# rafaelvp-db/databricks-distributed-deep-learning

Hardware: AMD Instinct MI355X
Metric: ResNet-50 images/sec (whole node) (higher is better)
Workload: dtype bf16

## Files before the change

### csrc/kernels/conv3_bwd.hip

```cpp
#include "ddl_lds.h"

#include <algorithm>

namespace {

constexpr int NW = 8, NTH = NW * 64;
constexpr int TM = 32;
constexpr int DPT = 6, SPT = 1;

struct C3Params {
    const bf16_t* dz;
    const bf16_t* x3;
    const float* mean3;
    const float* istd3;
    const float* coef3;
    const bf16_t* a2;
    const bf16_t* x2;
    const uint8_t* mask2;
    const float* mean2;
    const float* istd2;
    const bf16_t* wt;
    bf16_t* dz2;
    float* colstats;
    bf16_t* wpart;
    long M;
    int tiles, chunk;
    uint32_t dz2_bytes;
};

__device__ __forceinline__ u32x4 bn_apply8(bf16x8 dzv, bf16x8 xv, const float* A, const float* B, const float* D,
                                           bool valid) {
    const u32x4 gw = __builtin_bit_cast(u32x4, dzv), xw = __builtin_bit_cast(u32x4, xv);
    const uint32_t keep = valid ? ~0u : 0u;
    u32x4 o;
#pragma unroll
    for (int i = 0; i < 4; ++i) {
        const float g0 = lo_f(gw[i]), g1 = hi_f(gw[i]);
        const float x0 = lo_f(xw[i]), x1 = hi_f(xw[i]);
        const float o0 = bn_bwd_apply1(A[2 * i], g0, B[2 * i], x0, D[2 * i]);
        const float o1 = bn_bwd_apply1(A[2 * i + 1], g1, B[2 * i + 1], x1, D[2 * i + 1]);
        o[i] = pack2bf(o0, o1) & keep;
    }
    return o;
}

template <int CO, int CI, int NBUF>
__global__ __launch_bounds__(NTH, 1) void conv3_bwd_k(C3Params p) {
    static_assert(CO == 256 && CI == 64 && (NBUF == 2 || NBUF == 3), "shape");
    constexpr int WBYTES = CI * CO * 2, ZBYTES = TM * CO * 2, ABYTES = TM * CI * 2;
    constexpr int O_DZ = 0, O_X3 = ZBYTES, O_A2 = 2 * ZBYTES, O_X2 = O_A2 + ABYTES, O_MK = O_X2 + ABYTES;
    constexpr int BUFB = O_MK + 1024;
    constexpr int LDS = WBYTES + NBUF * BUFB;
    static_assert(LDS <= 160 * 1024, "LDS");
    __shared__ __attribute__((aligned(16))) char smem[LDS];
    const int tid = threadIdx.x, lane = tid & 63, wv = __builtin_amdgcn_readfirstlane(tid >> 6);
    const int g = lane >> 4, r16 = lane & 15;
    const uint32_t lds0 = (uint32_t)(uintptr_t)smem;
    const __amdgpu_buffer_rsrc_t crs = rsrc(p.dz2, p.dz2_bytes);
    const int t0 = blockIdx.x * p.chunk, t1 = min(p.tiles, t0 + p.chunk);

    auto prefetch = [&](int t, int buf) {
        char* base = smem + WBYTES + buf * BUFB;
        const long m0 = (long)t * TM;
#pragma unroll
        for (int qq = 0; qq < 2; ++qq) {
            const int q = qq * NW + wv, r = q * 2 + (lane >> 5), c = (lane & 31) ^ (r & 15);
            const long gr = min(m0 + r, p.M - 1);
            glds16_nt(p.dz + gr * CO + c * 8, base + O_DZ + q * 1024);
            glds16_nt(p.x3 + gr * CO + c * 8, base + O_X3 + q * 1024);
        }
        {
            const int q = wv & 3, r = q * 8 + (lane >> 3), c = (lane & 7) ^ (r & 7);
            const long gr = min(m0 + r, p.M - 1);
            glds16_nt((wv < 4 ? p.a2 : p.x2) + gr * CI + c * 8, base + (wv < 4 ? O_A2 : O_X2) + q * 1024);
        }
        {
            const long b = min(m0 * (CI / 8) + lane * 4, p.M * (CI / 8) - 4);
            const uint8_t* src = p.mask2 ? p.mask2 + b : (const uint8_t*)p.a2;
            glds4(src, base + O_MK);
        }
    };
#pragma unroll
    for (int qq = 0; qq < CI / 2 / NW; ++qq) {
        const int q = qq * NW + wv, r = q * 2 + (lane >> 5), c = (lane & 31) ^ (r & 15);
        glds16_nt(p.wt + (long)r * CO + c * 8, smem + q * 1024);
    }
#pragma unroll
    for (int u = 0; u < NBUF - 1; ++u)
        if (t0 + u < t1) prefetch(t0 + u, u);

    const int tc = tid & 31, tr = tid >> 5;
    float cA[8], cB[8], cD[8];
    bn_bwd_apply_coefs8(p.mean3, p.istd3, p.coef3, CO, tc * 8, cA, cB, cD);
    const uint32_t toff = tr * (CO * 2) + ((tc ^ tr) << 4);

    const int dj = wv & 3;
    const bool dgw = wv < 4;
    uint32_t aoff[2][CO / 32], boff[CO / 32];
#pragma unroll
    for (int kk = 0; kk < CO / 32; ++kk) {
        const int rb = 16 * dj + r16;
        boff[kk] = lds0 + rb * (CO * 2) + (((kk * 4 + g) ^ (rb & 15)) << 4);
#pragma unroll
        for (int i = 0; i < 2; ++i) {
            const int ra = 16 * i + r16;
            aoff[i][kk] = ra * (CO * 2) + (((kk * 4 + g) ^ (ra & 15)) << 4);
        }
    }
    uint32_t coff[2], moff[2];
#pragma unroll
    for (int i = 0; i < 2; ++i) {
        const int drow = 16 * i + r16;
        coff[i] = drow * (CI * 2) + (((2 * dj + (g >> 1)) ^ (drow & 7)) << 4) + (g & 1) * 8;
        moff[i] = drow * (CI / 8) + (dj >> 1) * 4;
    }
    const int mshift = (dj & 1) * 16 + 4 * g;
    float st_s[4] = {0.f, 0.f, 0.f, 0.f}, st_q[4] = {0.f, 0.f, 0.f, 0.f};

    const int q4 = (lane >> 2) & 3, pq = lane & 3;
    uint32_t wa[2][2], wb[4][2];
#pragma unroll
    for (int h = 0; h < 2; ++h) {
        const int r = 8 * g + q4 + 4 * h;
#pragma unroll
        for (int i = 0; i < 2; ++i) {
            const int col = 32 * wv + 16 * i + 4 * pq;
            wa[i][h] = r * (CO * 2) + (((col >> 3) ^ (r & 15)) << 4) + (pq & 1) * 8;
        }
#pragma unroll
        for (int j = 0; j < 4; ++j) {
            const int col = 16 * j + 4 * pq;
            wb[j][h] = r * (CI * 2) + (((col >> 3) ^ (r & 7)) << 4) + (pq & 1) * 8;
        }
    }
    f32x4 wacc[2][4];
#pragma unroll
    for (int i = 0; i < 2; ++i)
#pragma unroll
        for (int j = 0; j < 4; ++j) wacc[i][j] = (f32x4){0.f, 0.f, 0.f, 0.f};

    int buf = 0;
    for (int t = t0; t < t1; ++t) {
        wait_vm(min(NBUF - 1, t - t0) * SPT + min(NBUF - 2, t1 - 1 - t) * DPT);
        __builtin_amdgcn_s_barrier();
        if (t + NBUF - 1 < t1) prefetch(t + NBUF - 1, buf == 0 ? NBUF - 1 : buf - 1);
        const uint32_t img = lds0 + WBYTES + buf * BUFB;
        const long m0 = (long)t * TM;

        {
            const bf16x8 z0 = ds_read16(img + O_DZ + toff), z1 = ds_read16(img + O_DZ + toff + 16 * CO * 2);
            const bf16x8 x0 = ds_read16(img + O_X3 + toff), x1 = ds_read16(img + O_X3 + toff + 16 * CO * 2);
            LGKM0();
            __builtin_amdgcn_sched_barrier(0);
            ds_write16(img + O_DZ + toff, bn_apply8(z0, x0, cA, cB, cD, m0 + tr < p.M));
            ds_write16(img + O_DZ + toff + 16 * CO * 2, bn_apply8(z1, x1, cA, cB, cD, m0 + tr + 16 < p.M));
            LGKM0();
            __builtin_amdgcn_s_barrier();
        }

        f32x4 acc[2] = {{0.f, 0.f, 0.f, 0.f}, {0.f, 0.f, 0.f, 0.f}};
        if (dgw) {
#pragma unroll
            for (int k2 = 0; k2 < CO / 32; k2 += 4) {
                bf16x8 af[2][4], bfr[4];
#pragma unroll
                for (int u = 0; u < 4; ++u) {
                    af[0][u] = ds_read16(img + O_DZ + aoff[0][k2 + u]);
                    af[1][u] = ds_read16(img + O_DZ + aoff[1][k2 + u]);
                    bfr[u] = ds_read16(boff[k2 + u]);
                }
                LGKM0();
                __builtin_amdgcn_sched_barrier(0);
#pragma unroll
                for (int u = 0; u < 4; ++u) {
                    acc[0] = __builtin_amdgcn_mfma_f32_16x16x32_bf16(bfr[u], af[0][u], acc[0], 0, 0, 0);
                    acc[1] = __builtin_amdgcn_mfma_f32_16x16x32_bf16(bfr[u], af[1][u], acc[1], 0, 0, 0);
                }
                __builtin_amdgcn_sched_barrier(0);
            }
        }
        s16x4 fal[2][2], fbl[4][2];
#pragma unroll
        for (int h = 0; h < 2; ++h) {
#pragma unroll
            for (int i = 0; i < 2; ++i) fal[i][h] = ds_read_tr8(img + O_DZ + wa[i][h]);
#pragma unroll
            for (int j = 0; j < 4; ++j) fbl[j][h] = ds_read_tr8(img + O_A2 + wb[j][h]);
        }
        uint32_t mword[2] = {~0u, ~0u};
        uint2 ev[2] = {make_uint2(0u, 0u), make_uint2(0u, 0u)};
        if (dgw) {
#pragma unroll
            for (int i = 0; i < 2; ++i) {
                if (p.mask2) mword[i] = ds_read32(img + O_MK + moff[i]);
                ev[i] = ds_read8(img + O_X2 + coff[i]);
            }
        }
        LGKM0();
        __builtin_amdgcn_sched_barrier(0);
        {
            typedef short s16x8 __attribute__((ext_vector_type(8)));
            bf16x8 fa[2], fb[4];
#pragma unroll
            for (int i = 0; i < 2; ++i) {
                const s16x8 r = {fal[i][0][0], fal[i][0][1], fal[i][0][2], fal[i][0][3],
                                 fal[i][1][0], fal[i][1][1], fal[i][1][2], fal[i][1][3]};
                fa[i] = __builtin_bit_cast(bf16x8, r);
            }
#pragma unroll
            for (int j = 0; j < 4; ++j) {
                const s16x8 r = {fbl[j][0][0], fbl[j][0][1], fbl[j][0][2], fbl[j][0][3],
                                 fbl[j][1][0], fbl[j][1][1], fbl[j][1][2], fbl[j][1][3]};
                fb[j] = __builtin_bit_cast(bf16x8, r);
            }
#pragma unroll
            for (int i = 0; i < 2; ++i)
#pragma unroll
                for (int j = 0; j < 4; ++j)
                    wacc[i][j] = __builtin_amdgcn_mfma_f32_16x16x32_bf16(fb[j], fa[i], wacc[i][j], 0, 0, 0);
        }
        if (dgw) {
#pragma unroll
            for (int i = 0; i < 2; ++i) {
                float v[4] = {acc[i][0], acc[i][1], acc[i][2], acc[i][3]};
                const float xv[4] = {lo_f(ev[i].x), hi_f(ev[i].x), lo_f(ev[i].y), hi_f(ev[i].y)};
                const uint32_t bits = mword[i] >> mshift;
#pragma unroll
                for (int e = 0; e < 4; ++e) v[e] = ((bits >> e) & 1u) ? v[e] : 0.f;
                const uint32_t lo = pack2bf(v[0], v[1]), hi = pack2bf(v[2], v[3]);
                ds_write8(img + O_X2 + coff[i], make_uint2(lo, hi));
                if (m0 + 16 * i + r16 < p.M) {
                    const float tq[4] = {lo_f(lo), hi_f(lo), lo_f(hi), hi_f(hi)};
#pragma unroll
                    for (int e = 0; e < 4; ++e) {
                        st_s[e] += tq[e];
                        st_q[e] = __builtin_fmaf(tq[e], xv[e], st_q[e]);
                    }
                }
            }
        }
        LGKM0();
        __builtin_amdgcn_s_barrier();
        {
            const int row = 4 * wv + (lane >> 4), pc = lane & 15;
            const uint2 d = ds_read8(img + O_X2 + row * (CI * 2) + (((pc >> 1) ^ (row & 7)) << 4) + (pc & 1) * 8);
            LGKM0();
            __builtin_amdgcn_sched_barrier(0);
            const long grow = m0 + row;
            const uint32_t off = grow < p.M ? (uint32_t)((grow * CI + pc * 4) * 2) : 0x80000000u;
            __builtin_amdgcn_raw_buffer_store_b64(__builtin_bit_cast(u32x2, d), crs, (int)off, 0, 0);
        }
        buf = buf + 1 == NBUF ? 0 : buf + 1;
    }
    asm volatile("s_waitcnt vmcnt(0)" ::: "memory");
    __syncthreads();

    bf16_t* wout = p.wpart + (long)blockIdx.x * CO * CI;
#pragma unroll
    for (int i = 0; i < 2; ++i)
#pragma unroll
        for (int j = 0; j < 4; ++j)
            *reinterpret_cast<uint2*>(wout + (long)(32 * wv + 16 * i + r16) * CI + 16 * j + 4 * g) =
                make_uint2(pack2bf(wacc[i][j][0], wacc[i][j][1]), pack2bf(wacc[i][j][2], wacc[i][j][3]));

    if (dgw) {
#pragma unroll
        for (int e = 0; e < 4; ++e) {
            const float a = row16_sum(st_s[e]), b = row16_sum(st_q[e]);
            if (r16 == 0) {
                const int col = 16 * dj + 4 * g + e;
                p.colstats[(long)blockIdx.x * 2 * CI + col] = a;
                p.colstats[(long)blockIdx.x * 2 * CI + CI + col] =
                    __builtin_fmaf(-p.mean2[col], a, b) * p.istd2[col];
            }
        }
    }
}

}

DDL_API int ddl_conv3_bwd_grid(long M, int grid) {
    const int tiles64 = (int)((M + 63) / 64);
    const int g = std::min(grid > 0 ? std::min(grid, 256) : 256, tiles64);
    const int chunk64 = (tiles64 + g - 1) / g;
    return (tiles64 + chunk64 - 1) / chunk64;
}

DDL_API int ddl_conv3_bwd(const void* dz, const void* x3, const float* mean3, const float* istd3, const float* coef3,
                          const void* a2, const void* x2, const uint8_t* mask2, const float* mean2, const float* istd2,
                          const void* wt, void* dz2, float* colstats, void* wpart, long wpart_elems, void* dW,
                          int dw_f32, int accumulate, long M, int Cout, int Cin, int grid, hipStream_t st) {
    if (Cout != 256 || Cin != 64 || M < 1 || M * (long)Cout * 2 >= (1l << 31)) return -1;
    if (!dz || !x3 || !mean3 || !istd3 || !coef3 || !a2 || !x2 || !mean2 || !istd2 || !wt || !dz2 || !colstats ||
        !wpart || !dW)
        return -1;
    for (const void* q : {dz, x3, a2, x2, wt, (const void*)dz2, (const void*)wpart})
        if ((uintptr_t)q & 15) return -1;
    if ((uintptr_t)dW & (dw_f32 ? 15 : 7)) return -1;
    C3Params p{};
    p.dz = (const bf16_t*)dz;
    p.x3 = (const bf16_t*)x3;
    p.mean3 = mean3;
    p.istd3 = istd3;
    p.coef3 = coef3;
    p.a2 = (const bf16_t*)a2;
    p.x2 = (const bf16_t*)x2;
    p.mask2 = mask2;
    p.mean2 = mean2;
    p.istd2 = istd2;
    p.wt = (const bf16_t*)wt;
    p.dz2 = (bf16_t*)dz2;
    p.colstats = colstats;
    p.wpart = (bf16_t*)wpart;
    p.M = M;
    p.tiles = (int)((M + TM - 1) / TM);
    const int G = ddl_conv3_bwd_grid(M, grid);
    p.chunk = 2 * (((int)((M + 63) / 64) + G - 1) / G);
    p.dz2_bytes = (uint32_t)(M * Cin * 2);
    if (wpart_elems < (long)G * Cout * Cin) return -1;
    hipLaunchKernelGGL((conv3_bwd_k<256, 64, 3>), dim3(G), dim3(NTH), 0, st, p);
    ddl_wgrad_reduce(p.wpart, G, Cout, Cin, dW, Cin, accumulate, dw_f32, st);
    const hipError_t e = hipGetLastError();
    if (e != hipSuccess) return -2 - (int)e;
    return G;
}
```

### databricks_distributed_deep_learning_amd/ops/_lib.py

```python
from __future__ import annotations

import ctypes
import os
from typing import Optional

import torch

_PKG_DIR = os.path.dirname(os.path.dirname(os.path.abspath(__file__)))
LIB_PATH = os.environ.get("DDL_NATIVE_LIB") or os.path.join(_PKG_DIR, "_native", "libddl_kernels.so")

_lib: Optional[ctypes.CDLL] = None
_load_error: Optional[str] = None
_mode = os.environ.get("DDL_NATIVE", "auto").lower()


class NativeUnavailable(RuntimeError):
    pass


def set_mode(mode: str) -> None:
    global _mode
    if mode not in ("auto", "on", "off"):
        raise ValueError(mode)
    _mode = mode
# ... 40 lines not shown
    return _load_error


def use_native(*tensors: torch.Tensor) -> bool:
    if _mode == "off":
        return False
    if not all(t is None or t.is_cuda for t in tensors):
        return False
    if load() is None:
        raise NativeUnavailable(
            f"HIP kernel library unavailable on a GPU run: {_load_error}. "
            "Build it with `python csrc/build.py` or set DDL_NATIVE=off for stock PyTorch ops.")
    return True


def get() -> ctypes.CDLL:
    lib = load()
    if lib is None:
        raise NativeUnavailable(_load_error)
    return lib


def stream() -> ctypes.c_void_p:
    return ctypes.c_void_p(torch.cuda.current_stream().cuda_stream)


def ptr(t: Optional[torch.Tensor]) -> ctypes.c_void_p:
    return ctypes.c_void_p(0 if t is None else t.data_ptr())


def check(rc: int, what: str) -> None:
    if rc != 0:
        raise RuntimeError(f"native kernel {what} failed with HIP error {rc}")


P, I, L, F, U64 = ctypes.c_void_p, ctypes.c_int, ctypes.c_long, ctypes.c_float, ctypes.c_uint64
_SIGS = {
    "ddl_bn_stats_nblk": [L, I],
    "ddl_bn_bwd_nblk": [L, I],
    "ddl_bn_rows_sum": [P, I, I, P, P, P],
    "ddl_rows_sum_sink": [I, P, I, I, I, P, I, P, P],
    "ddl_bn_stats_partials": [I, P, L, I, P, P],
    "ddl_bn_bwd_partials": [I, P, P, P, P, P, L, I, I, P, P],
    "ddl_bn_bwd_finish": [I, P, P, P, P, P, P, L, L, I, I, P, P, P, P, P, P, P, I, P],
    "ddl_bn_bwd_from_partials": [I, P, I, P, L, P, P, P, P, P, L, I, P, P, P, P, P, I, P],
    "ddl_bn_partials_ws": [I, I],
    "ddl_bn_fwd_train": [I, P, L, I, P, P, P, P, F, F, P, P, P, P, P, P],
    "ddl_bn_eval_coeffs": [I, I, P, P, P, P, F, P, P, P],
    "ddl_bn_apply": [I, P, P, P, P, P, L, I, I, P, P],
    "ddl_bn_apply2": [I, P, P, P, P, P, P, P, L, I, I, P, P],
    "ddl_bn_relu_maxpool": [I, P, P, P, P, P, P, I, I, I, I, I, I, P],
    "ddl_bn_bwd_pool_nblk": [],
    "ddl_bn_bwd_pool": [I, P, P, P, P, P, P, P, I, I, I, I, I, I, P, P, P, P, P, I, P],
    "ddl_bn_bwd_coef_from_partials": [I, P, I, P, L, P, P, L, I, P, P, P, I, P],
    "ddl_bn_bwd_apply_coef": [I, P, P, P, P, P, L, I, P, P],
    "ddl_bn_fwd_from_partials": [I, P, I, L, I, P, P, P, P, F, F, P, P, P, P, P, L],
    "ddl_conv_w_dgrad": [P, P, I, I, I, I, I, I, P, P, P],
    "ddl_conv_w_dgrad_batch": [P, P, I, P],
    "ddl_gelu_bwd_colsum": [I, P, P, P, L, I, P, P, I, I, P],
    "ddl_acc_f32": [I, P, P, L, P],
    "ddl_tanh_bwd": [I, P, P, P, L, P],
    "ddl_copy2d": [I, P, L, L, L, P, L, L, L, P],
    "ddl_add_into": [I, P, P, L, P],
    "ddl_zero": [P, L, P],
    "ddl_rows_add_row": [I, P, P, P, L, L, P],
    "ddl_seq_prepend_add": [I, P, P, P, P, L, L, L, P],
    "ddl_sort_ids_ok": [L, L],
    "ddl_sort_ids": [P, L, P, P, P],
    "ddl_drain_acc": [I, P, P, L, P],
    "ddl_acc_grad": [I, P, P, L, I, I, P],
    "ddl_softmax_topk": [I, P, L, I, I, P, P, P, P],
    "ddl_gemm_conv_multi": [I, I, P, P, P, P, P, L, I, P, P],
    "ddl_conv3x3": [P, P, P, I, I, I, I, I, P, P, P, P, P, P, I, P],
    "ddl_conv3x3_wgrad": [P, P, P, I, I, I, I, I, P, L, I, I, I, P],
    "ddl_stem_wgrad": [P, P, P, I, I, I, I, I, I, I, P, L, I, I, I, P],
    "ddl_stem_fwd": [P, P, P, I, I, I, I, P, I, P],
    "ddl_s2d_input": [P, I, I, I, I, I, P, I, I, P],
    "ddl_s2d_weight": [P, I, I, I, I, P, I, I, P],
    "ddl_skinny_gemm": [P, P, P, L, I, I, P, P, P, P, P, P, I, P],
    "ddl_stream_gemm": [P, P, P, L, I, I, P, P, P, P, P, P, I, P],
    "ddl_stream_wgrad_ws": [I, I],
    "ddl_conv3_bwd_grid": [L, I],
    "ddl_conv3_bwd": [P, P, P, P, P, P, P, P, P, P, P, P, P, P, L, P, I, I, L, I, I, I, P],
    "ddl_bn_bwd": [I, P, P, P, P, P, P, L, I, I, P, P, P, P, P, P, I, P],
    "ddl_ln_supported": [I],
    "ddl_ln_fwd": [I, P, P, L, P, P, P, P, P, L, I, F, U64, F, P],
    "ddl_ln_bwd_nblk": [L],
    "ddl_ln_bwd": [I, P, P, P, L, P, P, P, P, P, P, P, L, I, I, P, U64, F, P, P, P, P],
    "ddl_gelu_fwd": [I, P, P, L, P],
    "ddl_gelu_bwd": [I, P, P, P, L, P],
    "ddl_dropout": [I, P, P, L, U64, F, P],
    "ddl_colsum_nblk": [L],
    "ddl_colsum": [I, P, L, I, P, P, I, I, P],
    "ddl_softmax_ce": [I, P, P, L, I, P, P, P, P],
    "ddl_scale_by": [I, P, P, P, L, P],
    "ddl_maxpool_fwd": [I, P, P, P, I, I, I, I, I, I, I, I, I, P],
    "ddl_maxpool_bwd": [I, P, P, P, I, I, I, I, I, I, I, I, I, P],
    "ddl_avgpool_fwd": [I, P, P, I, I, I, P],
    "ddl_avgpool_bwd": [I, P, P, I, I, I, P],
    "ddl_embedding_fwd": [I, P, P, P, L, I, P],
    "ddl_embedding_bwd": [I, P, P, P, P, L, L, I, I, P],
    "ddl_embedding_bwd_sorted": [I, P, P, P, P, P, L, I, I, P],
    "ddl_sgd_step": [I, P, P, I, P, P, P, I, P, F, F, F, I, I, P],
    "ddl_adamw_step": [I, P, P, I, P, P, P, P, I, P, F, F, F, F, F, F, F, F, F, P],
    "ddl_lamb_step": [I, P, P, I, P, P, P, P, I, P, F, F, F, F, F, F, F, F, F, P, P],
    "ddl_sumsq": [I, P, L, P, P],
    "ddl_lamb_phase1": [I, P, P, P, P, P, I, P, F, F, F, F, F, F, F, F, P, P],
    "ddl_lamb_phase2": [P, I, P, P, P, P, I, F, F, F, F, F, P, P],
}
_fns = {}


def fn(name: str):
    f = _fns.get(name)
    if f is None:
        f = getattr(get(), name)
        if name in _SIGS:
            f.argtypes = _SIGS[name]
        f.restype = ctypes.c_int
        _fns[name] = f
    return f


def call(name: str, *args) -> None:
    rc = fn(name)(*args, stream())
    if rc != 0:
        raise RuntimeError(f"native kernel {name} failed with code {rc}")


def register(sigs: dict) -> None:
    _SIGS.update(sigs)


def dcode(t: torch.Tensor) -> int:
    if t.dtype == torch.bfloat16:
        return 1
    if t.dtype == torch.float32:
        return 0
    raise TypeError(f"native kernels support fp32/bf16, got {t.dtype}")


def p(t: Optional[torch.Tensor]) -> int:
    return 0 if t is None else t.data_ptr()


def grad_sink(param) -> Optional[torch.Tensor]:
    if param is None:
        return None
    return getattr(param, "_ddl_main_grad", None)


def grad_ready(param) -> None:
    cb = getattr(param, "_ddl_grad_ready", None)
    if cb is not None:
        cb()


import contextlib as _contextlib

_WGRAD_STREAM = os.environ.get("DDL_WGRAD_STREAM", "0") != "0"
_side: dict = {}


def wgrad_stream_enabled() -> bool:
    return _WGRAD_STREAM

# ... 35 lines not shown
```

### databricks_distributed_deep_learning_amd/ops/_native_conv.py

```python
from __future__ import annotations

import ctypes
import os

import torch
import torch.nn.functional as F

from . import _lib
from ._lib import grad_ready, grad_sink
from ._native_gemm import MODE_CONV, MODE_CONVW, MODE_NN, MODE_NT, MODE_TN, gemm, plan, stats_rows_max
from ._native_norm import _BN_BWD_EPI, _BN_BWD_EPI_RES


def _desc(N, H, W, C, P, Q, stride, h_off, w_off, h_step, w_step, R, S, OH, OW, ostep=1, oa=0, ob=0):
    return [N, H, W, C, P, Q, stride, h_off, w_off, h_step, w_step, R, S, OH, OW, ostep, oa, ob]


STATS_MIN_K = int(os.environ.get("DDL_BN_STATS_MIN_K", "0"))
_DGRAD_NT = os.environ.get("DDL_DGRAD_NT", "1") != "0"


_CONV3X3 = os.environ.get("DDL_CONV3X3", "1") != "0"


# ... 313 lines not shown
            skey = "dgrad_path|" + "|".join(str(v) for v in key)
            planned = NG.lookup_choice(skey)
            if planned is not None and planned[0] in ("serial", "multi", "multi_narrow"):
                choice = _MULTI_CHOICE[key] = planned[0]
            else:
                choice = _pick_dgrad_path(key, serial, multi, dx)
                NG.record_choice(skey, (choice, 1))
        if choice == "serial":
            serial(dx)
        else:
            multi(dx, choice == "multi_narrow")
    else:
        serial(dx)
    return dx


_MULTI_CHOICE: dict = {}


def _pick_dgrad_path(key, serial, multi, dx):
    if not dx.is_cuda or torch.cuda.is_current_stream_capturing():
        return "serial"
    scratch = torch.empty_like(dx)
    serial(scratch)
    cands = {"serial": lambda: serial(scratch), "multi": lambda: multi(scratch, False),
             "multi_narrow": lambda: multi(scratch, True)}
    best, best_t = "serial", float("inf")
    for name, fn in cands.items():
        fn()
        e0, e1 = torch.cuda.Event(enable_timing=True), torch.cuda.Event(enable_timing=True)
        e0.record()
        for _ in range(5):
            fn()
        e1.record()
        e1.synchronize()
        t = e0.elapsed_time(e1)
        if t < best_t:
            best, best_t = name, t
    _MULTI_CHOICE[key] = best
    return best


def _direct3x3_wgrad(dy, x, dw, accumulate, grid=0):
    N, H, W_, C = x.shape
    if (tuple(dy.shape) != (N, H, W_, 64) or tuple(dw.shape) != (64, 3, 3, 64) or not dy.is_contiguous()
            or not x.is_contiguous() or not dw.is_contiguous() or dy.dtype != torch.bfloat16
            or x.dtype != torch.bfloat16 or dw.dtype not in (torch.bfloat16, torch.float32)):
        raise ValueError("direct 3x3 wgrad: operand shapes / layouts not covered")
    g = grid if grid > 0 else 256
    ws = torch.empty(g * 576 * 64, dtype=torch.float32, device=x.device)
    rc = _lib.fn("ddl_conv3x3_wgrad")(x.data_ptr(), dy.data_ptr(), dw.data_ptr(), N, H, W_, C, 64, ws.data_ptr(),
                                      ws.numel(), int(accumulate), int(dw.dtype == torch.float32), int(grid),
                                      _lib.stream())
    if rc != 0:
        raise RuntimeError(f"ddl_conv3x3_wgrad failed: {rc}")
    return dw


def _wgrad(dy, x, w_shape, stride, pad, out=None):
    N, H, W_, C = x.shape
    K, R, S, _ = w_shape
    _, P, Q, _ = dy.shape
    acc = out is not None
    dw = out if acc else torch.empty(K, R, S, C, dtype=dy.dtype, device=dy.device)
    if x.is_cuda and _direct3x3_ok(x.shape, w_shape, stride, pad) and dw.is_contiguous():
        return _direct3x3_wgrad(dy, x, dw, acc)
    M = N * P * Q
    if R == 1 and S == 1 and stride == 1 and pad == 0:
        gemm(MODE_TN, dy, K, x, C, dw, C, K, C, M, accumulate=acc)
    else:
        gemm(MODE_CONVW, dy, K, x, 0, dw, R * S * C, K, R * S * C, M, accumulate=acc,
             conv=_desc(N, H, W_, C, P, Q, stride, -pad, -pad, 1, 1, R, S, P, Q))
    return dw


def _conv3_fold_ok(x, w, stride, pad) -> bool:
    from . import bridge as B
    K, R, S, C = w.shape
    return (B.CONV3_FUSED and R == 1 and S == 1 and stride == 1 and pad == 0 and (K, C) in B.CONV3_SHAPES
            and x.is_cuda and x.dtype == torch.bfloat16 and w.dtype == torch.bfloat16 and x.is_contiguous()
            and w.is_contiguous() and x.numel() // C * K * 2 < 2 ** 31)


def _conv3_bwd_fused(parked, x, w, bnb, param, sink):
    dz, x3, mean3, istd3, coef = parked
    N, H, W_, C = x.shape
    K = w.shape[0]
    M = N * H * W_
    if (bnb is None or not _BN_BWD_EPI or tuple(bnb.x.shape) != tuple(x.shape) or not bnb.x.is_contiguous()
            or bnb.x.dtype != torch.bfloat16 or x3.numel() != M * K or dz.numel() != M * K
            or not dz.is_contiguous() or not x3.is_contiguous()
            or (bnb.mask is not None and bnb.mask.numel() * 8 < M * C)):
        return None
    if sink is not None and (not sink.is_contiguous() or sink.dtype not in (torch.bfloat16, torch.float32)):
        return None
    wt = _w_dgrad(w, [0], [0], param).view(C, K)
    dx = torch.empty(N, H, W_, C, dtype=x.dtype, device=x.device)
    dw = sink if sink is not None else torch.empty(K, 1, 1, C, dtype=x.dtype, device=x.device)
    G = _lib.fn("ddl_conv3_bwd_grid")(M, 0)
    part = torch.empty(max(stats_rows_max(M), 1024) * 2 * C + 64 * C, dtype=torch.float32, device=x.device)
    wpart = torch.empty(G * K * C, dtype=torch.bfloat16, device=x.device)
    rc = _lib.fn("ddl_conv3_bwd")(dz.data_ptr(), x3.data_ptr(), mean3.data_ptr(), istd3.data_ptr(), coef.data_ptr(),
                                  x.data_ptr(), bnb.x.data_ptr(), _lib.p(bnb.mask), bnb.mean.data_ptr(),
                                  bnb.istd.data_ptr(), wt.data_ptr(), dx.data_ptr(), part.data_ptr(),
                                  wpart.data_ptr(), wpart.numel(), dw.data_ptr(), int(dw.dtype == torch.float32),
                                  int(sink is not None), M, K, C, 0, _lib.stream())
    if rc == -1:
        return None
    if rc < 0:
        raise RuntimeError(f"ddl_conv3_bwd failed: {rc}")
    bnb.set(dx, part, rc)
    return dx, (None if sink is not None else dw)


def _conv3_materialise(parked, dy):
    from .bridge import Conv3Fold
    dz, x3, mean3, istd3, coef = parked
    C = x3.shape[-1]
    dx3 = torch.empty_like(x3)
    _lib.call("ddl_bn_bwd_apply_coef", 1, dz.data_ptr(), x3.data_ptr(), mean3.data_ptr(), istd3.data_ptr(),
              coef.data_ptr(), x3.numel() // C, C, dx3.data_ptr())
    if Conv3Fold.is_parked(parked, dy):
        return dx3
    return (dy - dz.view_as(dy)) + dx3.view_as(dy)


class _Conv(torch.autograd.Function):
    @staticmethod
    def forward(ctx, x, w, stride, pad, bridge=None, stats=None, grad_to=None):
        ctx.w_param = w
        ctx.bridge = bridge
        ctx.grad_to = grad_to
        ctx.c3 = None
        ctx.bnb = getattr(x, "_ddl_bnb", None) if grad_to is None else None
        x = x.contiguous()
        w = w.contiguous()
        ctx.stride, ctx.pad = stride, pad
        ctx.save_for_backward(x, w)
        y = _fwd(x, w, stride, pad, stats=stats)
        if _conv3_fold_ok(x, w, stride, pad) and y.is_contiguous():
            from .bridge import Conv3Fold
            ctx.c3 = y._ddl_c3 = Conv3Fold()
        return y

    @staticmethod
    def backward(ctx, dy):
        x, w = ctx.saved_tensors
        dy = dy.contiguous()
        dx = dw = None
        parked = ctx.c3.take() if ctx.c3 is not None else None
        if parked is not None:
            from .bridge import Conv3Fold
            if (Conv3Fold.is_parked(parked, dy) and ctx.needs_input_grad[0] and ctx.needs_input_grad[1]
                    and ctx.bridge is None and ctx.grad_to is None):
                sink = grad_sink(ctx.w_param)
                if sink is not None and sink.shape != w.shape:
                    sink = None
                out = _conv3_bwd_fused(parked, x, w, ctx.bnb, ctx.w_param, sink)
                if out is not None:
                    ctx.bnb = None
                    if sink is not None:
                        grad_ready(ctx.w_param)
                    return out[0], out[1], None, None, None, None, None
            dy = _conv3_materialise(parked, dy)
        del parked
        fork = _lib.fork_event() if ctx.needs_input_grad[1] else None
        if ctx.needs_input_grad[0]:
            res = ctx.bridge.take() if ctx.bridge is not None else None
            if res is not None:
                res = res.contiguous().view(x.shape)
            dx = _dgrad(dy, w, x.shape, ctx.stride, ctx.pad, residual=res, bnb=ctx.bnb, param=ctx.w_param)
            ctx.bnb = None
            if ctx.grad_to is not None and ctx.grad_to.offer(dx):
                dx = None
        if ctx.needs_input_grad[1]:
            sink = grad_sink(ctx.w_param)
            if sink is not None and sink.shape == w.shape:
                with _lib.side_stream(dy, x, after=fork):
                    _wgrad(dy, x, w.shape, ctx.stride, ctx.pad, out=sink)
                grad_ready(ctx.w_param)
            else:
                dw = _wgrad(dy, x, w.shape, ctx.stride, ctx.pad)
        return dx, dw, None, None, None, None, None


def _s2d_input(x, pad):
    N, H, W_, C = x.shape
    Hp, Wp = H + 2 * pad, W_ + 2 * pad
    Hp2, Wp2 = Hp + Hp % 2, Wp + Wp % 2
    if x.is_cuda and x.dtype == torch.bfloat16 and x.is_contiguous():
        xs = torch.empty(N, Hp2 // 2, Wp2 // 2, 16, dtype=x.dtype, device=x.device)
        _lib.call("ddl_s2d_input", x.data_ptr(), N, H, W_, C, pad, xs.data_ptr(), Hp2 // 2, Wp2 // 2)
        return xs
    xp = F.pad(x, (0, 4 - C, pad, pad + Wp2 - Wp, pad, pad + Hp2 - Hp))
    return xp.view(N, Hp2 // 2, 2, Wp2 // 2, 2, 4).permute(0, 1, 3, 2, 4, 5).reshape(N, Hp2 // 2, Wp2 // 2, 16)


def _s2d_weight(w):
    K, R, S, C = w.shape
    R2, S2 = (R + 1) // 2, (S + 1) // 2
    if w.is_cuda and w.dtype == torch.bfloat16 and w.is_contiguous():
        ws = torch.empty(K, R2, S2, 16, dtype=w.dtype, device=w.device)
        _lib.call("ddl_s2d_weight", w.data_ptr(), K, R, S, C, ws.data_ptr(), R2, S2)
        return ws
    wp = F.pad(w, (0, 4 - C, 0, 2 * S2 - S, 0, 2 * R2 - R))
    return wp.view(K, R2, 2, S2, 2, 4).permute(0, 1, 3, 2, 4, 5).reshape(K, R2, S2, 16)


def _s2d_weight_grad(dws, w_shape):
    K, R, S, C = w_shape
    R2, S2 = dws.shape[1], dws.shape[2]
    d = dws.view(K, R2, S2, 2, 2, 4).permute(0, 1, 3, 2, 4, 5).reshape(K, 2 * R2, 2 * S2, 4)
    return d[:, :R, :S, :C]


def _stem_wgrad_ok(xs, dy, ws_shape, w_shape) -> bool:
    if not (xs.is_cuda and dy.is_cuda):
        return False
    N, Hx, Wx, Cs = xs.shape
    _, P, Q, K = dy.shape
    return (tuple(ws_shape) == (64, 4, 4, 16) and Cs == 16 and K == 64 and Hx == P + 3 and Wx == Q + 3
            and P % 2 == 0 and Q % 16 == 0 and 16 <= Q <= 112 and w_shape[1] <= 8 and w_shape[2] <= 8
            and w_shape[3] <= 4 and xs.dtype == torch.bfloat16 and dy.dtype == torch.bfloat16
            and xs.is_contiguous() and dy.is_contiguous() and xs.data_ptr() % 16 == 0 and dy.data_ptr() % 16 == 0)


def _stem_wgrad(xs, dy, dw, accumulate, grid=0):
    N, _, _, _ = xs.shape
    _, P, Q, _ = dy.shape
    K, R, S, C = dw.shape
    g = grid if grid > 0 else 256
    ws = torch.empty(g * 64 * 256, dtype=torch.float32, device=xs.device)
    rc = _lib.fn("ddl_stem_wgrad")(xs.data_ptr(), dy.data_ptr(), dw.data_ptr(), N, P, Q, K, R, S, C, ws.data_ptr(),
                                   ws.numel(), int(accumulate), int(dw.dtype == torch.float32), int(grid),
                                   _lib.stream())
    if rc != 0:
        raise RuntimeError(f"ddl_stem_wgrad failed: {rc}")
    return dw


def _stem_fwd_ok(xs, ws) -> bool:
    if not xs.is_cuda:
        return False
    N, Hx, Wx, Cs = xs.shape
    P, Q = Hx - 3, Wx - 3
    return (tuple(ws.shape) == (64, 4, 4, 16) and Cs == 16 and P >= 4 and P % 4 == 0 and Q % 16 == 0
            and 16 <= Q <= 112 and xs.dtype == torch.bfloat16 and ws.dtype == torch.bfloat16
            and xs.is_contiguous() and ws.is_contiguous() and xs.data_ptr() % 16 == 0 and ws.data_ptr() % 16 == 0)


def _stem_fwd(xs, ws, stats=None, grid=0):
    N, Hx, Wx, _ = xs.shape
    P, Q = Hx - 3, Wx - 3
# ... 135 lines not shown
```

### databricks_distributed_deep_learning_amd/ops/_native_norm.py

```python
from __future__ import annotations

import os
from types import SimpleNamespace
from typing import Optional

import torch

from . import _lib
from ._native_elementwise import new_seed
from ._lib import call, dcode, grad_ready, grad_sink, p

_BN_BWD_EPI = os.environ.get("DDL_BN_BWD_EPI", "1") != "0"
_BN_BWD_EPI_RES = os.environ.get("DDL_BN_BWD_EPI", "1") not in ("0", "nores")


def _bn_supported(C: int) -> bool:
    return C % 8 == 0 and 256 % (C // 8) == 0


def _group_sum(row: torch.Tensor, group) -> None:
    import torch.distributed as dist
    from ..parallel import comm as _comm
    eng = _comm.active()
    if eng is not None and row.is_cuda and (group is None or group is dist.group.WORLD
# ... 23 lines not shown

class _BatchNormTrain(torch.autograd.Function):
    @staticmethod
    def forward(ctx, x, weight, bias, running_mean, running_var, momentum, eps, relu, residual, bridge=None,
                pre=None, group=None):
        ctx.bridge = bridge
        ctx.group = group
        ctx.c3 = _conv3_hint(x) if group is None else None
        x = x.contiguous()
        C = x.shape[-1]
        M = x.numel() // C
        dt = dcode(x)
        f32 = dict(dtype=torch.float32, device=x.device)
        stats = torch.empty(4, C, **f32)
        given = pre.take_for(x) if pre is not None else None
        if group is not None:
            import torch.distributed as dist
            world = dist.get_world_size(group)
            if given is not None:
                part, nblk = given
                ws = torch.empty(-(-nblk // 32) * 2 * C, **f32)
            else:
                nblk = _lib.fn("ddl_bn_stats_nblk")(M, C)
                part = torch.empty((nblk + -(-nblk // 32)) * 2 * C, **f32)
                call("ddl_bn_stats_partials", dt, p(x), M, C, p(part))
                ws = None
            row = torch.empty(2 * C, **f32)
            call("ddl_bn_rows_sum", p(part), nblk, 2 * C, p(row), p(ws))
            _group_sum(row, group)
            call("ddl_bn_fwd_from_partials", dt, p(row), 1, M * world, C, p(weight), p(bias), p(running_mean),
                 p(running_var), float(momentum), float(eps), p(stats[0]), p(stats[1]), p(stats[2]), p(stats[3]),
                 None, 0)
            ctx.m_total = M * world
        else:
            _bn_train_stats(x, weight, bias, running_mean, running_var, momentum, eps, given, stats)
        res = residual.contiguous() if residual is not None else None
        y = torch.empty_like(x)
        mask = torch.empty(x.numel() // 8, dtype=torch.uint8, device=x.device) if relu else None
        call("ddl_bn_apply", dt, p(x), p(res), p(stats[2]), p(stats[3]), p(y), x.numel(), C, int(relu), p(mask))
        ctx.relu = bool(relu)
        ctx.has_res = residual is not None
        ctx.params = (weight, bias)
        ctx.save_for_backward(x, mask, weight, stats)
        ctx.bnb = None
        if _BN_BWD_EPI and x.dtype == torch.bfloat16:
            from .bridge import BNBackward
            ctx.bnb = BNBackward(x, mask, stats[0], stats[1])
            y._ddl_bnb = ctx.bnb
        return y

    @staticmethod
    def backward(ctx, dy):
        x, mask, weight, stats = ctx.saved_tensors
        dx, dgamma, dbeta, dres = _bn_backward(ctx, dy, x, mask, weight, stats)
        return dx, dgamma, dbeta, None, None, None, None, None, dres, None, None, None


def _conv3_hint(x):
    hint = getattr(x, "_ddl_c3", None)
    if hint is None or not x.is_contiguous() or x.dtype != torch.bfloat16 or not x.requires_grad:
        return None
    return hint


def _bn_backward(ctx, dy, x, mask, weight, stats):
    dy = dy.contiguous()
    C = x.shape[-1]
    M = x.numel() // C
    nblk = _lib.fn("ddl_bn_bwd_nblk")(M, C)
    f32 = dict(dtype=torch.float32, device=x.device)
    part = torch.empty((nblk + -(-nblk // 32)) * 2 * C, **f32)
    coef = torch.empty(3 * C, **f32)
    sg, sb = grad_sink(ctx.params[0]), grad_sink(ctx.params[1])
    direct = sg is not None and sb is not None
    if direct:
        dgamma, dbeta = sg, sb
    else:
        dgamma = torch.empty_like(weight) if weight is not None else None
        dbeta = torch.empty_like(weight) if weight is not None else None
    given = ctx.bnb.take_for(dy) if ctx.bnb is not None else None
    ctx.bnb = None
    c3 = getattr(ctx, "c3", None)
    fold = c3 is not None and given is not None and ctx.group is None and weight is not None
    dx = None if fold else torch.empty_like(x)
    dres = torch.empty_like(x) if ctx.has_res and (given is None or ctx.group is not None) else None
    if given is not None:
        gpart, nrows = given
        if ctx.group is not None:
            row = torch.empty(2 * C, **f32)
            call("ddl_bn_rows_sum", p(gpart), nrows, 2 * C, p(row), None)
            local = row.clone()
            _group_sum(row, ctx.group)
            call("ddl_bn_bwd_finish", dcode(x), p(dy), None, p(x), p(stats[0]), p(stats[1]), p(weight), M,
                 ctx.m_total, C, 0, p(row), p(local), p(dgamma), p(dbeta), p(coef), p(dx), p(dres), int(direct))
        elif fold:
            ws = gpart[nrows * 2 * C:]
            call("ddl_bn_bwd_coef_from_partials", dcode(x), p(gpart), nrows, p(ws), ws.numel(), p(stats[1]),
                 p(weight), M, C, p(dgamma), p(dbeta), p(coef), int(direct))
            c3.park(dy, x, stats[0], stats[1], coef)
            dx = dy
            if ctx.has_res:
                dres = dy
        else:
            ws = gpart[nrows * 2 * C:]
            call("ddl_bn_bwd_from_partials", dcode(x), p(gpart), nrows, p(ws), ws.numel(), p(dy), p(x),
                 p(stats[0]), p(stats[1]), p(weight), M, C, p(dgamma), p(dbeta), p(coef), p(dx), None,
                 int(direct))
            if ctx.has_res:
                dres = dy
    elif ctx.group is not None:
        call("ddl_bn_bwd_partials", dcode(x), p(dy), p(mask), p(x), p(stats[0]), p(stats[1]), M, C,
             int(ctx.relu), p(part))
        row = torch.empty(2 * C, **f32)
        call("ddl_bn_rows_sum", p(part), nblk, 2 * C, p(row), None)
        local = row.clone()
        _group_sum(row, ctx.group)
        call("ddl_bn_bwd_finish", dcode(x), p(dy), p(mask), p(x), p(stats[0]), p(stats[1]), p(weight), M,
             ctx.m_total, C, int(ctx.relu), p(row), p(local), p(dgamma), p(dbeta), p(coef), p(dx), p(dres),
             int(direct))
    else:
        call("ddl_bn_bwd", dcode(x), p(dy), p(mask), p(x), p(stats[0]), p(stats[1]), p(weight), M, C,
             int(ctx.relu), p(part), p(dgamma), p(dbeta), p(coef), p(dx), p(dres), int(direct))
    if direct:
        grad_ready(ctx.params[0])
        grad_ready(ctx.params[1])
        dgamma = dbeta = None
    if dres is not None and ctx.bridge is not None:
        ctx.bridge.put(dres)
        dres = None
    return dx, dgamma, dbeta, dres


class _BatchNormAddBNTrain(torch.autograd.Function):

    @staticmethod
    def forward(ctx, x, weight, bias, running_mean, running_var, momentum, eps, x2, weight2, bias2, running_mean2,
                running_var2, momentum2, eps2, pre=None, pre2=None):
        ctx.c3 = _conv3_hint(x)
        x, x2 = x.contiguous(), x2.contiguous()
        C = x.shape[-1]
        f32 = dict(dtype=torch.float32, device=x.device)
        stats = torch.empty(4, C, **f32)
        stats2 = torch.empty(4, C, **f32)
        _bn_train_stats(x, weight, bias, running_mean, running_var, momentum, eps,
                        pre.take_for(x) if pre is not None else None, stats)
        _bn_train_stats(x2, weight2, bias2, running_mean2, running_var2, momentum2, eps2,
                        pre2.take_for(x2) if pre2 is not None else None, stats2)
        y = torch.empty_like(x)
        mask = torch.empty(x.numel() // 8, dtype=torch.uint8, device=x.device)
        call("ddl_bn_apply2", dcode(x), p(x), p(x2), p(stats[2]), p(stats[3]), p(stats2[2]), p(stats2[3]), p(y),
             x.numel(), C, 1, p(mask))
        ctx.bridge, ctx.group, ctx.relu, ctx.has_res = None, None, True, True
        ctx.params, ctx.params2 = (weight, bias), (weight2, bias2)
        ctx.save_for_backward(x, mask, weight, stats, x2, weight2, stats2)
        ctx.bnb = None
        if _BN_BWD_EPI and x.dtype == torch.bfloat16:
            from .bridge import BNBackward
            ctx.bnb = BNBackward(x, mask, stats[0], stats[1])
            y._ddl_bnb = ctx.bnb
        return y

    @staticmethod
    def backward(ctx, dy):
        x, mask, weight, stats, x2, weight2, stats2 = ctx.saved_tensors
        dx, dgamma, dbeta, dres = _bn_backward(ctx, dy, x, mask, weight, stats)
        c2 = SimpleNamespace(bnb=None, group=None, has_res=False, relu=False, params=ctx.params2, bridge=None)
        dx2, dgamma2, dbeta2, _ = _bn_backward(c2, dres, x2, None, weight2, stats2)
        return (dx, dgamma, dbeta, None, None, None, None, dx2, dgamma2, dbeta2, None, None, None, None, None, None)


class _BNReluMaxPoolTrain(torch.autograd.Function):

    @staticmethod
    def forward(ctx, x, weight, bias, running_mean, running_var, momentum, eps, pre=None):
        x = x.contiguous()
        N, H, W, C = x.shape
        P, Q = H // 2, W // 2
        stats = torch.empty(4, C, dtype=torch.float32, device=x.device)
        _bn_train_stats(x, weight, bias, running_mean, running_var, momentum, eps,
                        pre.take_for(x) if pre is not None else None, stats)
        y = torch.empty(N, P, Q, C, dtype=x.dtype, device=x.device)
        idx = torch.empty(N, P, Q, C, dtype=torch.uint8, device=x.device)
        mask = torch.empty(x.numel() // 8, dtype=torch.uint8, device=x.device)
        call("ddl_bn_relu_maxpool", dcode(x), p(x), p(stats[2]), p(stats[3]), p(y), p(idx), p(mask), N, H, W, C, P, Q)
        ctx.params = (weight, bias)
        ctx.save_for_backward(x, mask, weight, stats, idx)
        return y

    @staticmethod
    def backward(ctx, dy):
        x, mask, weight, stats, idx = ctx.saved_tensors
        N, H, W, C = x.shape
        dy = dy.contiguous()
        if not _FUSED_STEM_BWD:
            da = torch.empty_like(x)
            call("ddl_maxpool_bwd", dcode(dy), p(dy), p(idx), p(da), N, H, W, C, H // 2, W // 2, 3, 2, 1)
            c = SimpleNamespace(bnb=None, group=None, has_res=False, relu=True, params=ctx.params, bridge=None)
            dx, dgamma, dbeta, _ = _bn_backward(c, da, x, mask, weight, stats)
            return dx, dgamma, dbeta, None, None, None, None, None
        nblk = _lib.fn("ddl_bn_bwd_pool_nblk")()
        f32 = dict(dtype=torch.float32, device=x.device)
        part = torch.empty((nblk + -(-nblk // 32)) * 2 * C, **f32)
        coef = torch.empty(3 * C, **f32)
        dx = torch.empty_like(x)
        sg, sb = grad_sink(ctx.params[0]), grad_sink(ctx.params[1])
        direct = sg is not None and sb is not None
        dgamma, dbeta = (sg, sb) if direct else (torch.empty_like(weight), torch.empty_like(weight))
        call("ddl_bn_bwd_pool", dcode(x), p(dy), p(idx), p(mask), p(x), p(stats[0]), p(stats[1]), p(weight), N, H, W,
             C, H // 2, W // 2, p(part), p(dgamma), p(dbeta), p(coef), p(dx), int(direct))
        if direct:
            grad_ready(ctx.params[0])
            grad_ready(ctx.params[1])
            dgamma = dbeta = None
        return dx, dgamma, dbeta, None, None, None, None, None


def bn_relu_maxpool(x, weight, bias, running_mean, running_var, momentum, eps, pre=None):
    N, H, W, C = x.shape
    if (not _bn_supported(C) or x.dtype not in (torch.bfloat16, torch.float32)
            or H % 2 or W % 2 or weight is None):
        return None
    if weight.dtype != x.dtype:
        weight, bias = weight.to(x.dtype), bias.to(x.dtype)
    return _BNReluMaxPoolTrain.apply(x, weight, bias, running_mean, running_var, momentum, eps, pre)


_FUSED_STEM_BWD = os.environ.get("DDL_FUSED_STEM_BWD", "0") != "0"


def batch_norm_add_bn(x, weight, bias, running_mean, running_var, momentum, eps, x2, weight2, bias2,
                      running_mean2, running_var2, momentum2, eps2, pre=None, pre2=None):
    C = x.shape[-1]
    if (not _bn_supported(C) or x.dtype not in (torch.bfloat16, torch.float32) or x2.dtype != x.dtype
            or x2.shape != x.shape or weight is None or weight2 is None):
        return None
    if weight.dtype != x.dtype:
        weight, bias = weight.to(x.dtype), bias.to(x.dtype)
    if weight2.dtype != x.dtype:
        weight2, bias2 = weight2.to(x.dtype), bias2.to(x.dtype)
    return _BatchNormAddBNTrain.apply(x, weight, bias, running_mean, running_var, momentum, eps, x2, weight2, bias2,
                                      running_mean2, running_var2, momentum2, eps2, pre, pre2)


class _BatchNormEval(torch.autograd.Function):

    @staticmethod
    def forward(ctx, x, weight, bias, running_mean, running_var, eps, relu, residual):
        x = x.contiguous()
        C = x.shape[-1]
# ... 138 lines not shown
```

Before: 12870.

## Fuse residual-add epilogue into conv3 backward and fold downsample-branch BN backward

```diff
diff --git a/csrc/kernels/conv3_bwd.hip b/csrc/kernels/conv3_bwd.hip
--- a/csrc/kernels/conv3_bwd.hip
+++ b/csrc/kernels/conv3_bwd.hip
@@ -7,6 +7,7 @@
 constexpr int NW = 8, NTH = NW * 64;
 constexpr int TM = 32;
 constexpr int DPT = 6, SPT = 1;
+enum Epi { EPI_BNB = 0, EPI_RES = 1 };
 
 struct C3Params {
     const bf16_t* dz;
@@ -44,7 +45,7 @@
     return o;
 }
 
-template <int CO, int CI, int NBUF>
+template <int CO, int CI, int NBUF, int EPI>
 __global__ __launch_bounds__(NTH, 1) void conv3_bwd_k(C3Params p) {
     static_assert(CO == 256 && CI == 64 && (NBUF == 2 || NBUF == 3), "shape");
     constexpr int WBYTES = CI * CO * 2, ZBYTES = TM * CO * 2, ABYTES = TM * CI * 2;
@@ -192,7 +193,7 @@
         if (dgw) {
 #pragma unroll
             for (int i = 0; i < 2; ++i) {
-                if (p.mask2) mword[i] = ds_read32(img + O_MK + moff[i]);
+                if (EPI == EPI_BNB && p.mask2) mword[i] = ds_read32(img + O_MK + moff[i]);
                 ev[i] = ds_read8(img + O_X2 + coff[i]);
             }
         }
@@ -226,10 +227,10 @@
                 const float xv[4] = {lo_f(ev[i].x), hi_f(ev[i].x), lo_f(ev[i].y), hi_f(ev[i].y)};
                 const uint32_t bits = mword[i] >> mshift;
 #pragma unroll
-                for (int e = 0; e < 4; ++e) v[e] = ((bits >> e) & 1u) ? v[e] : 0.f;
+                for (int e = 0; e < 4; ++e) v[e] = EPI == EPI_RES ? v[e] + xv[e] : ((bits >> e) & 1u) ? v[e] : 0.f;
                 const uint32_t lo = pack2bf(v[0], v[1]), hi = pack2bf(v[2], v[3]);
                 ds_write8(img + O_X2 + coff[i], make_uint2(lo, hi));
-                if (m0 + 16 * i + r16 < p.M) {
+                if (EPI == EPI_BNB && m0 + 16 * i + r16 < p.M) {
                     const float tq[4] = {lo_f(lo), hi_f(lo), lo_f(hi), hi_f(hi)};
 #pragma unroll
                     for (int e = 0; e < 4; ++e) {
@@ -263,7 +264,7 @@
             *reinterpret_cast<uint2*>(wout + (long)(32 * wv + 16 * i + r16) * CI + 16 * j + 4 * g) =
                 make_uint2(pack2bf(wacc[i][j][0], wacc[i][j][1]), pack2bf(wacc[i][j][2], wacc[i][j][3]));
 
-    if (dgw) {
+    if (EPI == EPI_BNB && dgw) {
 #pragma unroll
         for (int e = 0; e < 4; ++e) {
             const float a = row16_sum(st_s[e]), b = row16_sum(st_q[e]);
@@ -286,15 +287,15 @@
     return (tiles64 + chunk64 - 1) / chunk64;
 }
 
-DDL_API int ddl_conv3_bwd(const void* dz, const void* x3, const float* mean3, const float* istd3, const float* coef3,
-                          const void* a2, const void* x2, const uint8_t* mask2, const float* mean2, const float* istd2,
-                          const void* wt, void* dz2, float* colstats, void* wpart, long wpart_elems, void* dW,
-                          int dw_f32, int accumulate, long M, int Cout, int Cin, int grid, hipStream_t st) {
+DDL_API int ddl_conv3_bwd_epi(const void* dz, const void* x3, const float* mean3, const float* istd3,
+                              const float* coef3, const void* a2, const void* x2, const uint8_t* mask2,
+                              const float* mean2, const float* istd2, const void* res, const void* wt, void* dz2,
+                              float* colstats, void* wpart, long wpart_elems, void* dW, int dw_f32, int accumulate,
+                              long M, int Cout, int Cin, int grid, hipStream_t st) {
     if (Cout != 256 || Cin != 64 || M < 1 || M * (long)Cout * 2 >= (1l << 31)) return -1;
-    if (!dz || !x3 || !mean3 || !istd3 || !coef3 || !a2 || !x2 || !mean2 || !istd2 || !wt || !dz2 || !colstats ||
-        !wpart || !dW)
-        return -1;
-    for (const void* q : {dz, x3, a2, x2, wt, (const void*)dz2, (const void*)wpart})
+    if (!dz || !x3 || !mean3 || !istd3 || !coef3 || !a2 || !wt || !dz2 || !wpart || !dW) return -1;
+    if (!res && (!x2 || !mean2 || !istd2 || !colstats)) return -1;
+    for (const void* q : {dz, x3, a2, res ? res : x2, wt, (const void*)dz2, (const void*)wpart})
         if ((uintptr_t)q & 15) return -1;
     if ((uintptr_t)dW & (dw_f32 ? 15 : 7)) return -1;
     C3Params p{};
@@ -304,8 +305,8 @@
     p.istd3 = istd3;
     p.coef3 = coef3;
     p.a2 = (const bf16_t*)a2;
-    p.x2 = (const bf16_t*)x2;
-    p.mask2 = mask2;
+    p.x2 = (const bf16_t*)(res ? res : x2);
+    p.mask2 = res ? nullptr : mask2;
     p.mean2 = mean2;
     p.istd2 = istd2;
     p.wt = (const bf16_t*)wt;
@@ -318,9 +319,18 @@
     p.chunk = 2 * (((int)((M + 63) / 64) + G - 1) / G);
     p.dz2_bytes = (uint32_t)(M * Cin * 2);
     if (wpart_elems < (long)G * Cout * Cin) return -1;
-    hipLaunchKernelGGL((conv3_bwd_k<256, 64, 3>), dim3(G), dim3(NTH), 0, st, p);
+    if (res) hipLaunchKernelGGL((conv3_bwd_k<256, 64, 3, EPI_RES>), dim3(G), dim3(NTH), 0, st, p);
+    else hipLaunchKernelGGL((conv3_bwd_k<256, 64, 3, EPI_BNB>), dim3(G), dim3(NTH), 0, st, p);
     ddl_wgrad_reduce(p.wpart, G, Cout, Cin, dW, Cin, accumulate, dw_f32, st);
     const hipError_t e = hipGetLastError();
     if (e != hipSuccess) return -2 - (int)e;
     return G;
 }
+
+DDL_API int ddl_conv3_bwd(const void* dz, const void* x3, const float* mean3, const float* istd3, const float* coef3,
+                          const void* a2, const void* x2, const uint8_t* mask2, const float* mean2, const float* istd2,
+                          const void* wt, void* dz2, float* colstats, void* wpart, long wpart_elems, void* dW,
+                          int dw_f32, int accumulate, long M, int Cout, int Cin, int grid, hipStream_t st) {
+    return ddl_conv3_bwd_epi(dz, x3, mean3, istd3, coef3, a2, x2, mask2, mean2, istd2, nullptr, wt, dz2, colstats,
+                             wpart, wpart_elems, dW, dw_f32, accumulate, M, Cout, Cin, grid, st);
+}
diff --git a/databricks_distributed_deep_learning_amd/ops/_lib.py b/databricks_distributed_deep_learning_amd/ops/_lib.py
--- a/databricks_distributed_deep_learning_amd/ops/_lib.py
+++ b/databricks_distributed_deep_learning_amd/ops/_lib.py
@@ -146,6 +146,7 @@
     "ddl_stream_wgrad_ws": [I, I],
     "ddl_conv3_bwd_grid": [L, I],
     "ddl_conv3_bwd": [P, P, P, P, P, P, P, P, P, P, P, P, P, P, L, P, I, I, L, I, I, I, P],
+    "ddl_conv3_bwd_epi": [P, P, P, P, P, P, P, P, P, P, P, P, P, P, P, L, P, I, I, L, I, I, I, P],
     "ddl_bn_bwd": [I, P, P, P, P, P, P, L, I, I, P, P, P, P, P, P, I, P],
     "ddl_ln_supported": [I],
     "ddl_ln_fwd": [I, P, P, L, P, P, P, P, P, L, I, F, U64, F, P],
diff --git a/databricks_distributed_deep_learning_amd/ops/_native_conv.py b/databricks_distributed_deep_learning_amd/ops/_native_conv.py
--- a/databricks_distributed_deep_learning_amd/ops/_native_conv.py
+++ b/databricks_distributed_deep_learning_amd/ops/_native_conv.py
@@ -419,15 +419,19 @@
             and w.is_contiguous() and x.numel() // C * K * 2 < 2 ** 31)
 
 
-def _conv3_bwd_fused(parked, x, w, bnb, param, sink):
+def _conv3_bwd_fused(parked, x, w, bnb, param, sink, res=None):
     dz, x3, mean3, istd3, coef = parked
     N, H, W_, C = x.shape
     K = w.shape[0]
     M = N * H * W_
-    if (bnb is None or not _BN_BWD_EPI or tuple(bnb.x.shape) != tuple(x.shape) or not bnb.x.is_contiguous()
-            or bnb.x.dtype != torch.bfloat16 or x3.numel() != M * K or dz.numel() != M * K
-            or not dz.is_contiguous() or not x3.is_contiguous()
-            or (bnb.mask is not None and bnb.mask.numel() * 8 < M * C)):
+    if x3.numel() != M * K or dz.numel() != M * K or not dz.is_contiguous() or not x3.is_contiguous():
+        return None
+    if res is not None:
+        if (bnb is not None or tuple(res.shape) != tuple(x.shape) or not res.is_contiguous()
+                or res.dtype != torch.bfloat16):
+            return None
+    elif (bnb is None or not _BN_BWD_EPI or tuple(bnb.x.shape) != tuple(x.shape) or not bnb.x.is_contiguous()
+            or bnb.x.dtype != torch.bfloat16 or (bnb.mask is not None and bnb.mask.numel() * 8 < M * C)):
         return None
     if sink is not None and (not sink.is_contiguous() or sink.dtype not in (torch.bfloat16, torch.float32)):
         return None
@@ -435,18 +439,24 @@
     dx = torch.empty(N, H, W_, C, dtype=x.dtype, device=x.device)
     dw = sink if sink is not None else torch.empty(K, 1, 1, C, dtype=x.dtype, device=x.device)
     G = _lib.fn("ddl_conv3_bwd_grid")(M, 0)
-    part = torch.empty(max(stats_rows_max(M), 1024) * 2 * C + 64 * C, dtype=torch.float32, device=x.device)
     wpart = torch.empty(G * K * C, dtype=torch.bfloat16, device=x.device)
-    rc = _lib.fn("ddl_conv3_bwd")(dz.data_ptr(), x3.data_ptr(), mean3.data_ptr(), istd3.data_ptr(), coef.data_ptr(),
-                                  x.data_ptr(), bnb.x.data_ptr(), _lib.p(bnb.mask), bnb.mean.data_ptr(),
-                                  bnb.istd.data_ptr(), wt.data_ptr(), dx.data_ptr(), part.data_ptr(),
-                                  wpart.data_ptr(), wpart.numel(), dw.data_ptr(), int(dw.dtype == torch.float32),
-                                  int(sink is not None), M, K, C, 0, _lib.stream())
+    if res is not None:
+        part = None
+        epi = (None, None, None, None, res.data_ptr())
+    else:
+        part = torch.empty(max(stats_rows_max(M), 1024) * 2 * C + 64 * C, dtype=torch.float32, device=x.device)
+        epi = (bnb.x.data_ptr(), _lib.p(bnb.mask), bnb.mean.data_ptr(), bnb.istd.data_ptr(), None)
+    rc = _lib.fn("ddl_conv3_bwd_epi")(dz.data_ptr(), x3.data_ptr(), mean3.data_ptr(), istd3.data_ptr(),
+                                      coef.data_ptr(), x.data_ptr(), *epi, wt.data_ptr(), dx.data_ptr(), _lib.p(part),
+                                      wpart.data_ptr(), wpart.numel(), dw.data_ptr(),
+                                      int(dw.dtype == torch.float32), int(sink is not None), M, K, C, 0,
+                                      _lib.stream())
     if rc == -1:
         return None
     if rc < 0:
-        raise RuntimeError(f"ddl_conv3_bwd failed: {rc}")
-    bnb.set(dx, part, rc)
+        raise RuntimeError(f"ddl_conv3_bwd_epi failed: {rc}")
+    if bnb is not None:
+        bnb.set(dx, part, rc)
     return dx, (None if sink is not None else dw)
 
 
@@ -486,14 +496,25 @@
         dy = dy.contiguous()
         dx = dw = None
         parked = ctx.c3.take() if ctx.c3 is not None else None
+        res, took = None, False
         if parked is not None:
             from .bridge import Conv3Fold
             if (Conv3Fold.is_parked(parked, dy) and ctx.needs_input_grad[0] and ctx.needs_input_grad[1]
-                    and ctx.bridge is None and ctx.grad_to is None):
+                    and ctx.grad_to is None):
+                if ctx.bridge is not None:
+                    res, took = ctx.bridge.take(), True
+                    if res is not None:
+                        res = res.contiguous().view(x.shape)
+                fuse = ctx.bridge is None or (res is not None and ctx.bnb is None)
                 sink = grad_sink(ctx.w_param)
                 if sink is not None and sink.shape != w.shape:
                     sink = None
-                out = _conv3_bwd_fused(parked, x, w, ctx.bnb, ctx.w_param, sink)
+                if not fuse:
+                    out = None
+                elif res is None:
+                    out = _conv3_bwd_fused(parked, x, w, ctx.bnb, ctx.w_param, sink)
+                else:
+                    out = _conv3_bwd_fused(parked, x, w, None, ctx.w_param, sink, res=res)
                 if out is not None:
                     ctx.bnb = None
                     if sink is not None:
@@ -503,9 +524,10 @@
         del parked
         fork = _lib.fork_event() if ctx.needs_input_grad[1] else None
         if ctx.needs_input_grad[0]:
-            res = ctx.bridge.take() if ctx.bridge is not None else None
-            if res is not None:
-                res = res.contiguous().view(x.shape)
+            if not took:
+                res = ctx.bridge.take() if ctx.bridge is not None else None
+                if res is not None:
+                    res = res.contiguous().view(x.shape)
             dx = _dgrad(dy, w, x.shape, ctx.stride, ctx.pad, residual=res, bnb=ctx.bnb, param=ctx.w_param)
             ctx.bnb = None
             if ctx.grad_to is not None and ctx.grad_to.offer(dx):
diff --git a/databricks_distributed_deep_learning_amd/ops/_native_norm.py b/databricks_distributed_deep_learning_amd/ops/_native_norm.py
--- a/databricks_distributed_deep_learning_amd/ops/_native_norm.py
+++ b/databricks_distributed_deep_learning_amd/ops/_native_norm.py
@@ -129,7 +129,9 @@
     ctx.bnb = None
     c3 = getattr(ctx, "c3", None)
     fold = c3 is not None and given is not None and ctx.group is None and weight is not None
-    dx = None if fold else torch.empty_like(x)
+    fold_red = (c3 is not None and given is None and ctx.group is None and weight is not None
+                and not ctx.relu and not ctx.has_res and x.dtype == torch.bfloat16)
+    dx = None if fold or fold_red else torch.empty_like(x)
     dres = torch.empty_like(x) if ctx.has_res and (given is None or ctx.group is not None) else None
     if given is not None:
         gpart, nrows = given
@@ -165,6 +167,13 @@
         call("ddl_bn_bwd_finish", dcode(x), p(dy), p(mask), p(x), p(stats[0]), p(stats[1]), p(weight), M,
              ctx.m_total, C, int(ctx.relu), p(row), p(local), p(dgamma), p(dbeta), p(coef), p(dx), p(dres),
              int(direct))
+    elif fold_red:
+        call("ddl_bn_bwd_partials", dcode(x), p(dy), None, p(x), p(stats[0]), p(stats[1]), M, C, 0, p(part))
+        ws = part[nblk * 2 * C:]
+        call("ddl_bn_bwd_coef_from_partials", dcode(x), p(part), nblk, p(ws), ws.numel(), p(stats[1]), p(weight),
+             M, C, p(dgamma), p(dbeta), p(coef), int(direct))
+        c3.park(dy, x, stats[0], stats[1], coef)
+        dx = dy
     else:
         call("ddl_bn_bwd", dcode(x), p(dy), p(mask), p(x), p(stats[0]), p(stats[1]), p(weight), M, C,
              int(ctx.relu), p(part), p(dgamma), p(dbeta), p(coef), p(dx), p(dres), int(direct))
@@ -184,6 +193,7 @@
     def forward(ctx, x, weight, bias, running_mean, running_var, momentum, eps, x2, weight2, bias2, running_mean2,
                 running_var2, momentum2, eps2, pre=None, pre2=None):
         ctx.c3 = _conv3_hint(x)
+        ctx.c3_2 = _conv3_hint(x2)
         x, x2 = x.contiguous(), x2.contiguous()
         C = x.shape[-1]
         f32 = dict(dtype=torch.float32, device=x.device)
@@ -211,7 +221,8 @@
     def backward(ctx, dy):
         x, mask, weight, stats, x2, weight2, stats2 = ctx.saved_tensors
         dx, dgamma, dbeta, dres = _bn_backward(ctx, dy, x, mask, weight, stats)
-        c2 = SimpleNamespace(bnb=None, group=None, has_res=False, relu=False, params=ctx.params2, bridge=None)
+        c2 = SimpleNamespace(bnb=None, group=None, has_res=False, relu=False, params=ctx.params2, bridge=None,
+                             c3=ctx.c3_2)
         dx2, dgamma2, dbeta2, _ = _bn_backward(c2, dres, x2, None, weight2, stats2)
         return (dx, dgamma, dbeta, None, None, None, None, dx2, dgamma2, dbeta2, None, None, None, None, None, None)
 
```

Measured after the change: 12990 (median of 6 runs). No clear change (+1.0%).
